# Terascale-All-sensing-Research-Studio/MOV-SLAM

Measured on AMD Instinct MI355X. Metric: local-BA iterations/sec (50 KF x 20k MapPoint window), higher is better.
Workload: dtype f64; 1 GPU; LocalBundleAdjustment 50 KF + 10 fixed x 20000 MapPoints, E=110510 mono edges, Huber on, 10 LM iterations (cfg3, seed 1003); one window per GPU; parallelism=1 window

## Files before the change

### mov-slam_amd/csrc/coarse_level.h

```cpp
#pragma once
#include <hip/hip_runtime.h>

#include <type_traits>

#include "device_math.h"
#include "device_types.h"
#include "handoff.h"

namespace movba {

#ifndef MOVBA_COARSE_EXTRAPOLATE
#define MOVBA_COARSE_EXTRAPOLATE 1
#endif

template <int kT, int kNC, int kPA>
__device__ __forceinline__ void coarse_build(const DevWindow &w, const PcgParams &pp, int trial, double lambda, double *sm, bool extrapolate)
{
    double *Ac = sm;
    double *gj = Ac + kNC * kNC;
    int &s_bad = *reinterpret_cast<int *>(gj + 9 * kNC + 2);
    const int tid = threadIdx.x;
    const int nf = w.nfree;
#ifdef MOVBA_CLOCK_STAMP
    unsigned long long cst_last = __builtin_amdgcn_s_memtime();
#define COARSE_STAMP(k) do { const unsigned long long _t = __builtin_amdgcn_s_memtime(); if (tid == 0) w.ctrl->dbg_seg2[k] += _t - cst_last; cst_last = _t; } while (0)
#else
#define COARSE_STAMP(k) do { } while (0)
#endif
    const double *part = w.part, *part_ = part;
    double *blocks = w.blocks_c;
    if (tid == 0) s_bad = 0;
    for (int idx = tid; idx < kNC * kNC; idx += kT) Ac[idx] = 0.0;

    const int ndiag = nf * 36;
    for (int idx = tid; idx < w.n_multi * 36; idx += kT) {
        const int m = idx / 36, k = idx - m * 36, pr = w.multi_pairs[m];
        double sacc = 0.0;
        for (int itx = w.pair_item_start[pr]; itx < w.pair_item_start[pr + 1]; ++itx) sacc += part[(size_t)itx * kPartStride + k];
        blocks[pr * 36 + k] = -sacc;
    }
    for (int base = tid; base < ndiag; base += 4 * kT) {
        int k[4], hu[4], i0[4], i1[4];
        double s[4] = { 0, 0, 0, 0 }, hp[4] = { 0, 0, 0, 0 };
        int nmax = 0;
#pragma unroll
        for (int m = 0; m < 4; ++m) {
            const int idx = min(base + m * kT, ndiag - 1);
            const int pr = idx / 36;
            k[m] = idx - pr * 36;
            const int a = k[m] / 6, b = k[m] - a * 6;
            hu[m] = 42 + (a <= b ? ut6(a, b) : ut6(b, a));
            i0[m] = w.pair_item_start[pr]; i1[m] = w.pair_item_start[pr + 1];
            nmax = max(nmax, i1[m] - i0[m]);
        }
        for (int o = 0; o < nmax; o += 6) {
            double sv[4][6], hv[4][6];
#pragma unroll
            for (int m = 0; m < 4; ++m)
#pragma unroll
                for (int u = 0; u < 6; ++u) {
                    const double *src = part + (size_t)min(i0[m] + o + u, i1[m] - 1) * kPartStride;
                    sv[m][u] = src[k[m]]; hv[m][u] = src[hu[m]];
                }
#pragma unroll
            for (int m = 0; m < 4; ++m)
#pragma unroll
                for (int u = 0; u < 6; ++u) { const bool in = i0[m] + o + u < i1[m]; s[m] += in ? sv[m][u] : 0.0; hp[m] += in ? hv[m][u] : 0.0; }
        }
#pragma unroll
        for (int m = 0; m < 4; ++m) {
            const int idx = base + m * kT;
            if (idx < ndiag) blocks[idx] = (hp[m] + ((k[m] % 7 == 0) ? lambda : 0.0)) - s[m];
        }
    }
    __syncthreads();
    COARSE_STAMP(2);
    double *aggc = gj;
    if (tid < kNC / kPA) {
        const int g0 = pp.wave_row0[tid], g1 = pp.wave_row0[tid + 1];
        aggc[tid] = g0 + 0.5 * (g1 - g0 - 1); aggc[kNC / kPA + tid] = 1.0 / fmax(1.0, 0.5 * (g1 - g0));
    }
    int *tent = reinterpret_cast<int *>(gj + 9 * kNC + 8), *tij = tent + w.cblk_ptr[w.n_cblk];
    for (int q = tid; q < w.cblk_ptr[w.n_cblk]; q += kT) { tent[q] = w.cblk_ent[q]; tij[q] = w.cblk_ij[q]; }
    __syncthreads();
    const int nw = w.n_cblk * 6;
    const bool split = 2 * nw <= kT;
    auto walk = [&](int cb, int a, int part, double (&s00)[6], double (&s01)[6], double (&s10)[6], double (&s11)[6]) {
        const int g = w.cblk_g[cb], h = w.cblk_h[cb];
        const double cg = aggc[g], ch = aggc[h], ig = aggc[kNC / kPA + g], ih = aggc[kNC / kPA + h];
        int t0 = w.cblk_ptr[cb], t1 = w.cblk_ptr[cb + 1];
        if (split) {
            const int n = t1 - t0, front = min(n, (((n + 1) >> 1) + 7) & ~7);
            if (part == 0) t1 = t0 + front; else t0 += front;
        }
#pragma unroll
        for (int m = 0; m < 6; ++m) s00[m] = s01[m] = s10[m] = s11[m] = 0.0;
        for (int t = t0; t < t1; t += 8) {
            int pk[8], ij[8];
            double v[8][6];
#pragma unroll
            for (int u = 0; u < 8; ++u) { const int tt = min(t + u, t1 - 1); pk[u] = tent[tt]; ij[u] = tij[tt]; }
#pragma unroll
            for (int u = 0; u < 8; ++u) {
                const int e = pk[u];
                const double *src = (e & 1) ? part_ + (size_t)(e >> 2) * kPartStride : blocks + (size_t)(e >> 2) * 36;
                const int o0 = (e & 2) ? a : a * 6, st = (e & 2) ? 6 : 1;
#pragma unroll
                for (int m = 0; m < 6; ++m) v[u][m] = src[o0 + st * m];
            }
#pragma unroll
            for (int u = 0; u < 8; ++u) {
                const bool in = t + u < t1;
                const double sgn = in ? ((pk[u] & 1) ? -1.0 : 1.0) : 0.0;
                const double pi = ((ij[u] >> 16) - cg) * ig, pj = ((ij[u] & 0xffff) - ch) * ih;
#pragma unroll
                for (int m = 0; m < 6; ++m) {
                    const double x = sgn * v[u][m];
                    s00[m] += x; s01[m] += pj * x; s10[m] += pi * x; s11[m] += pi * pj * x;
                }
            }
        }
        return Ac + (g * kPA + a) * kNC + h * kPA;
    };
    if (split) {
        const bool active = tid < 2 * nw;
        const int half = tid >= nw, wi = tid - half * nw;
        double s00[6], s01[6], s10[6], s11[6];
        double *dst = nullptr;
        if (active) dst = walk(wi / 6, wi - (wi / 6) * 6, half, s00, s01, s10, s11);
        if (active && !half) {
#pragma unroll
            for (int m = 0; m < 6; ++m) { dst[m] = s00[m]; dst[6 + m] = s01[m]; dst[6 * kNC + m] = s10[m]; dst[6 * kNC + 6 + m] = s11[m]; }
        }
        __syncthreads();
        if (active && half) {
#pragma unroll
            for (int m = 0; m < 6; ++m) { dst[m] += s00[m]; dst[6 + m] += s01[m]; dst[6 * kNC + m] += s10[m]; dst[6 * kNC + 6 + m] += s11[m]; }
        }
    } else {
        for (int wi = tid; wi < nw; wi += kT) {
            double s00[6], s01[6], s10[6], s11[6];
            double *dst = walk(wi / 6, wi - (wi / 6) * 6, 0, s00, s01, s10, s11);
#pragma unroll
            for (int m = 0; m < 6; ++m) { dst[m] = s00[m]; dst[6 + m] = s01[m]; dst[6 * kNC + m] = s10[m]; dst[6 * kNC + 6 + m] = s11[m]; }
        }
    }
    __syncthreads();
    if (tid < kNC) {
        const int g = tid / kPA, d = (tid - g * kPA) / 6, nrows = pp.wave_row0[g + 1] - pp.wave_row0[g];
        if (nrows == 0 || (d == 1 && nrows < 2)) {
            for (int j = 0; j < kNC; ++j) { Ac[tid * kNC + j] = 0.0; Ac[j * kNC + tid] = 0.0; }
        }
    }
    __syncthreads();
    if (tid < kNC) {
        const int g = tid / kPA, d = (tid - g * kPA) / 6, nrows = pp.wave_row0[g + 1] - pp.wave_row0[g];
        if (nrows == 0 || (d == 1 && nrows < 2)) Ac[tid * kNC + tid] = 1.0;
    }
    __syncthreads();
    if (extrapolate) {
        double *prev = w.ac_prev;
        const double lam_prev = prev[kNC * kNC], trial_prev = prev[kNC * kNC + 1];
        double gamma = 0.0;
        if (trial >= 1 && trial_prev == (double)(trial - 1) && lambda != lam_prev && MOVBA_COARSE_EXTRAPOLATE) {
            gamma = (lambda * (1.0 / 3.0) - lambda) / (lambda - lam_prev);
            gamma = fmin(fmax(gamma, -1.0), 1.0 / 3.0);
            if (!isfinite(gamma)) gamma = 0.0;
        }
        constexpr int kPer = kNC * kNC / kT;
        static_assert(kPer * kT == kNC * kNC, "one pass");
        double pv[kPer];
#pragma unroll
        for (int u = 0; u < kPer; ++u) pv[u] = prev[tid + u * kT];
        __syncthreads();
#pragma unroll
        for (int u = 0; u < kPer; ++u) {
            const double a = Ac[tid + u * kT];
            prev[tid + u * kT] = a;
            if (gamma != 0.0) Ac[tid + u * kT] = a + gamma * (a - pv[u]);
        }
        if (tid == 0) { prev[kNC * kNC] = lambda; prev[kNC * kNC + 1] = (double)trial; }
        __syncthreads();
    }

    COARSE_STAMP(3);
    static_assert(kNC == 96 && kT == 512, "tile layout written for 96 x 96 on 512 threads");
    double *dsc = gj + 8 * kNC + 2;
    double *pvs = gj + 8 * kNC;
    if (tid < kNC) { const double d = Ac[tid * kNC + tid]; dsc[tid] = (d > 0.0 && isfinite(d)) ? rsqrt(d) : 0.0; if (!(d > 0.0) || !isfinite(d)) s_bad = 1; }
    __syncthreads();
    const int rg = tid >> 4, cg = tid & 15;
    double t[3][6];
#pragma unroll
    for (int r = 0; r < 3; ++r)
#pragma unroll
        for (int q = 0; q < 6; ++q) t[r][q] = Ac[(3 * rg + r) * kNC + 6 * cg + q] * dsc[3 * rg + r] * dsc[6 * cg + q];
    unsigned live = 0;
    for (int q = 0; q < kNC / 6; ++q) {
        const int nrows = pp.wave_row0[(q >> 1) + 1] - pp.wave_row0[q >> 1];
        if (!(nrows == 0 || ((q & 1) && nrows < 2))) live |= 1u << q;
    }
    __syncthreads();
    auto publish = [&](auto Ctag, int gq, int buf) {
        constexpr int C = decltype(Ctag)::value;
        constexpr int lr0 = C % 3, lr1 = (C + 1) % 3;
        const int rg0 = 2 * gq + C / 3, rg1 = 2 * gq + (C + 1) / 3;
        double *R1 = gj + buf * 4 * kNC, *C1 = R1 + kNC, *R2 = C1 + kNC, *C2 = R2 + kNC;
        if (rg == rg0) {
#pragma unroll
            for (int q = 0; q < 6; ++q) R1[6 * cg + q] = t[lr0][q] + ((cg == gq && q == C) ? 1.0 : 0.0);
        }
        if (rg == rg1) {
#pragma unroll
            for (int q = 0; q < 6; ++q) R2[6 * cg + q] = t[lr1][q];
        }
        if (cg == gq) {
#pragma unroll
            for (int r = 0; r < 3; ++r) { C1[3 * rg + r] = t[r][C] - ((rg == rg0 && r == lr0) ? 1.0 : 0.0); C2[3 * rg + r] = t[r][C + 1]; }
        }
        if (rg == rg0 && cg == gq) pvs[buf] = t[lr0][C];
    };
    int kk = live ? __builtin_ctz(live) : kNC / 6;
    if (kk < kNC / 6) publish(std::integral_constant<int, 0>{}, kk, 0);
    __syncthreads();
    bool bad = s_bad != 0;
    int buf = 0;
    auto pair_step = [&](auto Ctag, int gq) -> bool {
        constexpr int C = decltype(Ctag)::value;
        constexpr int lr1 = (C + 1) % 3;
        const int k = 6 * gq + C, rg1 = 2 * gq + (C + 1) / 3;
        const double *R1 = gj + buf * 4 * kNC, *C1 = R1 + kNC, *R2 = C1 + kNC, *C2 = R2 + kNC;
        const double p1 = pvs[buf];
        const double o12 = R1[k + 1], o21 = C1[k + 1], q22 = R2[k + 1];
        double r1[6], r2[6], c1[3], c2[3];
#pragma unroll
        for (int q = 0; q < 6; ++q) { r1[q] = R1[6 * cg + q]; r2[q] = R2[6 * cg + q]; }
#pragma unroll
        for (int r = 0; r < 3; ++r) { c1[r] = C1[3 * rg + r]; c2[r] = C2[3 * rg + r]; }
        if (!(p1 > 0.0) || !isfinite(p1)) return false;
        double ip1 = __builtin_amdgcn_rcp(p1);
        ip1 = ip1 * (2.0 - p1 * ip1);
        ip1 = ip1 * (2.0 - p1 * ip1);
        const double s12 = o12 * ip1;
        const double p2 = q22 - o21 * s12;
        if (!(p2 > 0.0) || !isfinite(p2)) return false;
        double ip2 = __builtin_amdgcn_rcp(p2);
        ip2 = ip2 * (2.0 - p2 * ip2);
        ip2 = ip2 * (2.0 - p2 * ip2);
#pragma unroll
        for (int q = 0; q < 6; ++q) {
            r1[q] *= ip1;
            r2[q] = ((r2[q] - o21 * r1[q]) + ((cg == gq && q == C + 1) ? 1.0 : 0.0)) * ip2;
        }
#pragma unroll
        for (int r = 0; r < 3; ++r) c2[r] = (c2[r] - c1[r] * s12) - ((rg == rg1 && r == lr1) ? 1.0 : 0.0);
#pragma unroll
        for (int r = 0; r < 3; ++r)
#pragma unroll
            for (int q = 0; q < 6; ++q) { t[r][q] -= c1[r] * r1[q]; t[r][q] -= c2[r] * r2[q]; }
        return true;
    };
    while (kk < kNC / 6 && !bad) {
        const unsigned later = kk < 31 ? (live & ~((2u << kk) - 1u)) : 0u;
        const int next = later ? __builtin_ctz(later) : kNC / 6;
        if (!pair_step(std::integral_constant<int, 0>{}, kk)) { bad = true; break; }
        publish(std::integral_constant<int, 2>{}, kk, buf ^ 1);
        __syncthreads(); buf ^= 1;
        if (!pair_step(std::integral_constant<int, 2>{}, kk)) { bad = true; break; }
        publish(std::integral_constant<int, 4>{}, kk, buf ^ 1);
        __syncthreads(); buf ^= 1;
        if (!pair_step(std::integral_constant<int, 4>{}, kk)) { bad = true; break; }
        if (next < kNC / 6) publish(std::integral_constant<int, 0>{}, next, buf ^ 1);
        __syncthreads(); buf ^= 1;
        kk = next;
    }
    if (bad && tid == 0) s_bad = 1;
    __syncthreads();
    COARSE_STAMP(4);
    float *dst = w.aci + (size_t)(trial & 1) * kNC * kNC;
#pragma unroll
    for (int r = 0; r < 3; ++r)
#pragma unroll
        for (int q = 0; q < 6; ++q) dst[(3 * rg + r) * kNC + 6 * cg + q] = (float)(t[r][q] * dsc[3 * rg + r] * dsc[6 * cg + q]);
    __syncthreads();
    if (tid == 0) w.aci_tag[trial & 1] = s_bad ? -1 : trial;
    COARSE_STAMP(5);
}

}
```

### mov-slam_amd/csrc/pcg_kernel.hip

```cpp
#include <hip/hip_runtime.h>

#include "coarse_level.h"
#include "device_math.h"
#include "device_types.h"
#include "handoff.h"
#include "kernels.h"

namespace movba {

#ifdef MOVBA_CLOCK_STAMP
#define SEG_STAMP(k) do { unsigned long long _t; asm volatile("s_memtime %0\n\ts_waitcnt lgkmcnt(0)" : "=s"(_t) :: "memory"); seg[k] += _t - seg_last; seg_last = _t; } while (0)
#else
#define SEG_STAMP(k) do { } while (0)
#endif
#ifdef MOVBA_CLOCK_STAMP
#define SETUP_STAMP(k) do { const unsigned long long _t = __builtin_amdgcn_s_memtime(); if (tid == 0) c->dbg_seg2[k] += _t - setup_last; setup_last = _t; } while (0)
#else
#define SETUP_STAMP(k) do { } while (0)
#endif

#ifdef MOVBA_PCG_NO_UNIFORM
#define PCG_UNI(x) (x)
#else
#define PCG_UNI(x) uniform_f64(x)
#endif

namespace {

constexpr int kT = kPcgRowsThreads;
constexpr int kNW = kT / 64;
constexpr int kOwnBatch = 10;
constexpr int kPA = kCoarsePerAgg;
constexpr int kNC = kPA * kNW;
static_assert(kNC == kCoarseDim, "coarse dimension");

__device__ __forceinline__ double sum_fixed(const double *red)
{
    static_assert(kNW == 8, "tree written for 8 waves");
    const double2 *r2 = reinterpret_cast<const double2 *>(red);
    const double2 a = r2[0], b = r2[1], c = r2[2], d = r2[3];
    return ((a.x + a.y) + (b.x + b.y)) + ((c.x + c.y) + (d.x + d.y));
}

}

template <bool OVERFLOW, bool PADDED>
__device__ __forceinline__ void pcg_rows_body(const DevWindow &w, const PcgParams &pp, int trial, int role)
{
    static_assert(!(OVERFLOW && PADDED), "the padded layout holds the register-resident pairs only");
    extern __shared__ __attribute__((aligned(16))) double sm[];
    Ctrl *c = w.ctrl;
    const int tid = threadIdx.x, ln = tid & 63;
    const int wv = __builtin_amdgcn_readfirstlane(tid >> 6);
    const bool fresh = pp.use_coarse == 2;
    const bool solver = role == 0 && !fresh;
    const int nf = w.nfree, n = 6 * nf;
    const int b0 = pp.wave_row0[wv], b1 = pp.wave_row0[wv + 1];
    const int row = b0 * 6 + ln;
    const bool owner = ln < 6 * (b1 - b0);
    const int bi = owner ? row / 6 : 0, ba = owner ? row - bi * 6 : 0;
    const int ctrial = fresh ? trial : trial - 1;
    int cur = 0;
    double lambda = 0.0;
#ifdef MOVBA_CLOCK_STAMP
    const unsigned long long stamp_c0 = __builtin_amdgcn_s_memtime(), stamp_t0 = __builtin_amdgcn_s_memrealtime();
    unsigned long long setup_last = stamp_c0;
#endif
    const double *part = w.part;
    if (!solver) {
        if (c->done) return;
        cur = c->cur; lambda = c->lambda;
        if (role == 1) {
            coarse_build<kT, kNC, kPA>(w, pp, trial, lambda, sm, true);
            return;
        }
        coarse_build<kT, kNC, kPA>(w, pp, trial, lambda, sm, false);
        __syncthreads();
    }
    int done_w = 0;
    if (solver) { done_w = c->done; cur = c->cur; lambda = c->lambda; }
    int aci_tag = -1;
    if (pp.use_coarse) {
        typedef __attribute__((address_space(1))) const void *gptr_t;
        typedef __attribute__((address_space(3))) void *lptr_t;
        const int npad0 = (6 * w.nfree + 1) & ~1;
        float *acf0 = reinterpret_cast<float *>(sm + 2 * npad0 + 36 * w.nfree + 2 * kNW + 2);
        aci_tag = w.aci_tag[max(ctrial, 0) & 1];
        const float *src = w.aci + (size_t)(max(ctrial, 0) & 1) * kNC * kNC;
        static_assert((kNC * kNC) % 256 == 0, "whole waves of 16-byte pieces");
#pragma unroll
        for (int u = 0; u * kT * 4 < kNC * kNC; ++u) {
            const int piece = tid + u * kT;
            if ((piece & ~63) * 4 < kNC * kNC)
                __builtin_amdgcn_global_load_lds((gptr_t)(src + 4 * piece), (lptr_t)(acf0 + 4 * (piece & ~63)), 16, 0, 0);
        }
    }
    const int4 *plan = reinterpret_cast<const int4 *>(w.lane_plan) + (size_t)tid * 3;
    const int4 pl0 = plan[0], pl1 = plan[1], plo = plan[2];
    const int oi0 = plo.x, oi1 = plo.y;
    const int rp_b0 = pp.wave_ent0[wv], rp_b1 = pp.wave_ent0[wv + 1], rp_nf = pp.nrowent, rp_bi = plo.z, rp_bi1 = plo.w;
    constexpr int kRecFly = 4;
    double2 rv[kRecFly][4];
    const double2 *rec0 = reinterpret_cast<const double2 *>(w.rec_d + (size_t)bi * w.rec_slots * 48 + ba * 8);
#pragma unroll
    for (int u = 0; u < kRecFly; ++u) {
        const double2 *src = rec0 + (size_t)min(u, w.rec_slots - 1) * 24;
#pragma unroll
        for (int q = 0; q < 4; ++q) rv[u][q] = src[q];
    }
    double Bo[2][36];
    if (!OVERFLOW) {
#pragma unroll
        for (int k = 0; k < 2; ++k)
#pragma unroll
            for (int q = 0; q < 36; ++q) Bo[k][q] = w.img_b[(size_t)(36 * k + q) * kT + tid];
    }
    if (solver && done_w) return;
    SETUP_STAMP(6);
    const int npad = (n + 1) & ~1;
    const int nrowent_all = rp_nf;

    double *p_lds = sm;
    double *r_lds = p_lds + npad;
    double *minv = r_lds + npad;
    double *red0 = minv + 36 * nf;
    double *red1 = red0 + kNW;
    float *Acf = reinterpret_cast<float *>(red1 + kNW + 2);
    double *rcg = red1 + kNW + 2 + kNC * kNC / 2;
    double *zstrip = rcg + kNC + 32 * wv;
    double *ustrip = zstrip + 16;
    double z_reg = 0.0, u_reg = 0.0;
    double *ypart = rcg + kNC + 32 * kNW;
    constexpr int kYDummy = 5 * kOwnBatch + 6;
    const int ypart_len = PADDED ? n * kOwnBatch + kYDummy + kOwnBatch : 6 * ((nrowent_all >> 1) + 1 + kOwnBatch);
    double *sdiag = ypart + ypart_len;
    double *rsw = sdiag + 36 * nf + 64 * wv;
    if (PADDED) {
        for (int k = tid; k < ypart_len; k += kT) ypart[k] = 0.0;
    }
    const int nrowent = nrowent_all;
    const int P0 = rp_b0 >> 1, P1 = rp_b1 >> 1;
    const int own_p0 = rp_bi >> 1, own_p1 = rp_bi1 >> 1;
    const int own_cnt = own_p1 - own_p0;
    const int nb = b1 - b0;

    if (OVERFLOW) {
        const int e0 = 2 * (P0 + 64), ntail = max(2 * P1 - e0, 0) * 36;
        for (int base = ln; base < ntail; base += 8 * 64) {
            int q[8], src[8], hu[8], i0[8], i1[8], pr[8];
            double sv[8], hv[8];
#pragma unroll
            for (int u = 0; u < 8; ++u) {
                const int idx = min(base + 64 * u, ntail - 1);
                const int e = e0 + idx / 36;
                q[u] = idx - (idx / 36) * 36;
                const RowEnt re = w.row_ent[e];
                const int a = q[u] / 6, b = q[u] - a * 6;
                pr[u] = re.block;
                src[u] = re.transposed ? b * 6 + a : q[u];
                hu[u] = 42 + (a <= b ? ut6(a, b) : ut6(b, a));
                i0[u] = re.block >= 0 ? w.pair_item_start[re.block] : 0;
                i1[u] = re.block >= 0 ? w.pair_item_start[re.block + 1] : 0;
            }
#pragma unroll
            for (int u = 0; u < 8; ++u) {
                const double *rec = part + (size_t)i0[u] * kPartStride;
                sv[u] = i1[u] > i0[u] ? rec[src[u]] : 0.0;
                hv[u] = (i1[u] > i0[u] && pr[u] < nf) ? rec[hu[u]] : 0.0;
            }
#pragma unroll
            for (int u = 0; u < 8; ++u)
                for (int itx = i0[u] + 1; itx < i1[u]; ++itx) {
                    const double *rec = part + (size_t)itx * kPartStride;
                    sv[u] += rec[src[u]];
                    if (pr[u] < nf) hv[u] += rec[hu[u]];
                }
#pragma unroll
            for (int u = 0; u < 8; ++u) {
                const int idx = base + 64 * u;
                if (idx < ntail) {
                    const bool dg = pr[u] >= 0 && pr[u] < nf;
                    w.blocks_ov[(size_t)e0 * 36 + idx] = dg ? (hv[u] + (q[u] % 7 == 0 ? lambda : 0.0)) - sv[u] : -sv[u];
                }
            }
        }
        __syncthreads();
    }

    int colo[2];
    const int my_pair = P0 + ln;
    const bool have_pair = my_pair < P1;
    int yslot = (have_pair ? my_pair : (nrowent >> 1)) * 6;
    const double *yown = ypart + own_p0 * 6 + ba;
    if (PADDED) {
        yslot = n * kOwnBatch;
#pragma unroll
        for (int u = 0; u < 10; ++u) {
            const int q0 = __builtin_amdgcn_readlane(rp_bi, 6 * u) >> 1, q1 = __builtin_amdgcn_readlane(rp_bi1, 6 * u) >> 1;
            if (u < nb && have_pair && my_pair >= q0 && my_pair < q1) yslot = (b0 + u) * 6 * kOwnBatch + (my_pair - q0);
        }
        yown = ypart + (owner ? row : 0) * kOwnBatch;
    }
    double r_r = 0.0;
    double mi[6] = { 1, 1, 1, 1, 1, 1 };
    auto wave_lds_sync0 = [&]() {
        __builtin_amdgcn_fence(__ATOMIC_RELEASE, "wavefront");
        __builtin_amdgcn_wave_barrier();
        __builtin_amdgcn_fence(__ATOMIC_ACQUIRE, "wavefront");
    };
    if (owner) {
        double d6[6] = { 0, 0, 0, 0, 0, 0 }, cc = 0.0, bb = 0.0;
        const int ni = oi1 - oi0;
        auto add = [&](const double2 (&v)[4], bool in) {
            d6[0] += in ? v[0].x : 0.0; d6[1] += in ? v[0].y : 0.0; d6[2] += in ? v[1].x : 0.0;
            d6[3] += in ? v[1].y : 0.0; d6[4] += in ? v[2].x : 0.0; d6[5] += in ? v[2].y : 0.0;
            cc += in ? v[3].x : 0.0; bb += in ? v[3].y : 0.0;
        };
#pragma unroll
        for (int u = 0; u < kRecFly; ++u) add(rv[u], u < ni);
        for (int i0 = kRecFly; i0 < ni; i0 += kRecFly) {
            double2 v[kRecFly][4];
#pragma unroll
            for (int u = 0; u < kRecFly; ++u) {
                const double2 *src = rec0 + (size_t)min(i0 + u, ni - 1) * 24;
#pragma unroll
                for (int q = 0; q < 4; ++q) v[u][q] = src[q];
            }
#pragma unroll
            for (int u = 0; u < kRecFly; ++u) add(v[u], i0 + u < ni);
        }
#pragma unroll
        for (int q = 0; q < 6; ++q) d6[q] += q == ba ? lambda : 0.0;
#pragma unroll
        for (int q = 0; q < 6; ++q) sdiag[bi * 36 + ba * 6 + q] = d6[q];
        r_r = bb - cc;
        w.bp[row] = bb;
#pragma unroll
        for (int q = 0; q < 6; ++q) mi[q] = d6[q];
    }
    SETUP_STAMP(7);
    {
        bool bad = false;
#pragma unroll
        for (int k = 0; k < 6; ++k) {
            double *strip = ((k & 1) ? p_lds : r_lds) + (owner ? bi * 6 : 0);
            if (owner && ba == k) {
                const double p = mi[k];
                if (!(p > 0.0)) bad = true;
                double pinv = __builtin_amdgcn_rcp(p);
                pinv = pinv * (2.0 - p * pinv);
                pinv = pinv * (2.0 - p * pinv);
#pragma unroll
                for (int q = 0; q < 6; ++q) { mi[q] = q == k ? pinv : mi[q] * pinv; strip[q] = mi[q]; }
            }
            wave_lds_sync0();
            if (owner && ba != k) {
                const double2 *sr = reinterpret_cast<const double2 *>(strip);
                const double2 s0 = sr[0], s1 = sr[1], s2 = sr[2];
                const double srow[6] = { s0.x, s0.y, s1.x, s1.y, s2.x, s2.y };
                const double f = mi[k];
#pragma unroll
                for (int q = 0; q < 6; ++q) mi[q] = q == k ? -f * srow[k] : mi[q] - f * srow[q];
            }
        }
        if (owner) {
#pragma unroll
            for (int q = 0; q < 6; ++q) minv[bi * 36 + ba * 6 + q] = mi[q];
        }
        wave_lds_sync0();
        if (owner) {
            double col[6];
#pragma unroll
            for (int q = 0; q < 6; ++q) col[q] = minv[bi * 36 + q * 6 + ba];
#pragma unroll
            for (int q = 0; q < 6; ++q) mi[q] = 0.5 * (mi[q] + col[q]);
        }
        wave_lds_sync0();
        if (owner) {
#pragma unroll
            for (int q = 0; q < 6; ++q) minv[bi * 36 + ba * 6 + q] = mi[q];
        }
        const int wbad = __any(bad) ? 1 : 0;
        if (ln == 0) reinterpret_cast<int *>(red1)[wv] = wbad;
    }
    const bool coarse = pp.use_coarse && ctrial >= 0 && aci_tag == ctrial;
    SETUP_STAMP(0);
    wave_lds_sync0();

#pragma unroll
    for (int k = 0; k < 2; ++k) {
        colo[k] = 0;
        const int4 pl = k ? pl1 : pl0;
        const bool valid = pl.x >= 0, tr = valid && ((pl.y >> 30) & 1) != 0;
        if (valid) colo[k] = pl.y & 0x3fffffff;
        const bool diag = valid && pl.x < nf, from_img = !OVERFLOW && valid && pl.x >= nf && pl.w - pl.z == 1;
        if (!OVERFLOW) {
#pragma unroll
            for (int q = 0; q < 36; ++q) Bo[k][q] = from_img ? -Bo[k][q] : 0.0;
        } else {
#pragma unroll
            for (int q = 0; q < 36; ++q) Bo[k][q] = 0.0;
        }
        if (diag) {
            const double2 *src = reinterpret_cast<const double2 *>(sdiag + pl.x * 36);
#pragma unroll
            for (int q = 0; q < 18; ++q) { const double2 v = src[q]; Bo[k][2 * q] = v.x; Bo[k][2 * q + 1] = v.y; }
        }
        if (__any(valid && !diag && !from_img)) {
            double raw[36];
#pragma unroll
            for (int q = 0; q < 36; ++q) raw[q] = 0.0;
            const bool mine = valid && !diag && !from_img;
            for (int itx = mine ? pl.z : 0; itx < (mine ? pl.w : 0); ++itx) {
                const double2 *src = reinterpret_cast<const double2 *>(part + (size_t)itx * kPartStride);
#pragma unroll
                for (int q = 0; q < 18; ++q) { const double2 v = src[q]; raw[2 * q] -= v.x; raw[2 * q + 1] -= v.y; }
            }
#pragma unroll
            for (int a = 0; a < 6; ++a)
#pragma unroll
                for (int q = 0; q < 6; ++q) Bo[k][a * 6 + q] = mine ? (tr ? raw[q * 6 + a] : raw[a * 6 + q]) : Bo[k][a * 6 + q];
        }
    }
    SETUP_STAMP(1);

    double x_r = 0.0, z_r = 0.0;
    const double2 *mrow = reinterpret_cast<const double2 *>(minv + (owner ? bi * 36 + ba * 6 : 0));
    const double2 *rblk = reinterpret_cast<const double2 *>(PADDED ? rsw + (owner ? (bi - b0) * 6 : 0) : r_lds + (owner ? bi * 6 : 0));
    auto wave_lds_sync = [&]() {
        __builtin_amdgcn_fence(__ATOMIC_RELEASE, "wavefront");
        __builtin_amdgcn_wave_barrier();
        __builtin_amdgcn_fence(__ATOMIC_ACQUIRE, "wavefront");
    };
    const double agg_c = uniform_f64(b0 + 0.5 * (nb - 1)), agg_ih = uniform_f64(1.0 / fmax(1.0, 0.5 * nb));
    const double agg_cc = uniform_f64(0.5 * (nb - 1));
    const double phi = owner ? (bi - agg_c) * agg_ih : 0.0;
    const int crow = min(ln >> 2, kPA - 1), cq = ln & 3;
    auto restrict_own = [&](double v_r) {
        if (PADDED) rsw[ln] = owner ? v_r : 0.0;
        else if (owner) r_lds[row] = v_r;
        wave_lds_sync();
        if (ln < kPA) {
            const int a = ln < 6 ? ln : ln - 6;
            const double *rb = PADDED ? rsw + a : r_lds + b0 * 6 + a;
            double v[10];
#pragma unroll
            for (int u = 0; u < 10; ++u) v[u] = rb[6 * u];
            if (!PADDED) {
#pragma unroll
                for (int u = 0; u < 10; ++u) v[u] = (u < nb) ? v[u] : 0.0;
            }
            const double tc = (((v[0] + v[1]) + (v[2] + v[3])) + ((v[4] + v[5]) + (v[6] + v[7]))) + (v[8] + v[9]);
            const double ti = (((v[1] + 2.0 * v[2]) + (3.0 * v[3] + 4.0 * v[4])) + ((5.0 * v[5] + 6.0 * v[6]) + (7.0 * v[7] + 8.0 * v[8]))) + 9.0 * v[9];
            rcg[wv * kPA + ln] = ln < 6 ? tc : (ti - agg_cc * tc) * agg_ih;
        }
    };
    const int ra = ln < kPA ? (ln < 6 ? ln : ln - 6) : 0;
    auto restrict_issue = [&](double v_r, double (&v)[10]) {
        if (PADDED) rsw[ln] = owner ? v_r : 0.0;
        else if (owner) r_lds[row] = v_r;
        wave_lds_sync();
        const double *rb = PADDED ? rsw + ra : r_lds + b0 * 6 + ra;
#pragma unroll
        for (int u = 0; u < 10; ++u) v[u] = rb[6 * u];
    };
    auto restrict_finish = [&](double (&v)[10]) {
        if (ln < kPA) {
            if (!PADDED) {
#pragma unroll
                for (int u = 0; u < 10; ++u) v[u] = (u < nb) ? v[u] : 0.0;
            }
            const double tc = (((v[0] + v[1]) + (v[2] + v[3])) + ((v[4] + v[5]) + (v[6] + v[7]))) + (v[8] + v[9]);
            const double ti = (((v[1] + 2.0 * v[2]) + (3.0 * v[3] + 4.0 * v[4])) + ((5.0 * v[5] + 6.0 * v[6]) + (7.0 * v[7] + 8.0 * v[8]))) + 9.0 * v[9];
            rcg[wv * kPA + ln] = ln < 6 ? tc : (ti - agg_cc * tc) * agg_ih;
        }
    };
    auto coarse_rows = [&]() {
        const float4 *arow = reinterpret_cast<const float4 *>(Acf + (wv * kPA + crow) * kNC + cq * 24);
        const double2 *rcv = reinterpret_cast<const double2 *>(rcg + cq * 24);
        double t0 = 0.0, t1 = 0.0;
#pragma unroll
        for (int q = 0; q < 6; q += 2) {
            const float4 a0 = arow[q], a1 = arow[q + 1];
            const double2 c0 = rcv[2 * q], c1 = rcv[2 * q + 1], c2 = rcv[2 * q + 2], c3 = rcv[2 * q + 3];
            t0 += ((double)a0.x * c0.x + (double)a0.y * c0.y) + ((double)a0.z * c1.x + (double)a0.w * c1.y);
            t1 += ((double)a1.x * c2.x + (double)a1.y * c2.y) + ((double)a1.z * c3.x + (double)a1.w * c3.y);
        }
        double t = t0 + t1;
        t += dpp_mov0<0xb1>(t);
        t += dpp_mov0<0x4e>(t);
        return t;
    };
    if (coarse) {
        restrict_own(r_r);
        u_reg = 0.0;
        __syncthreads();
        const double t = coarse_rows();
        z_reg = t;
        __syncthreads();
    } else __syncthreads();
    int anybad = 0;
#pragma unroll
    for (int k = 0; k < kNW; ++k) anybad |= reinterpret_cast<const int *>(red1)[k];
    auto precond = [&](double rv) {
        if (PADDED) rsw[ln] = owner ? rv : 0.0;
        else if (owner) r_lds[row] = rv;
        wave_lds_sync();
        const double2 m0 = mrow[0], m1 = mrow[1], m2 = mrow[2];
        const double2 r0 = rblk[0], r1 = rblk[1], r2 = rblk[2];
        double s = (m0.x * r0.x + m0.y * r0.y) + (m1.x * r1.x + m1.y * r1.y) + (m2.x * r2.x + m2.y * r2.y);
        if (fresh && coarse) s = 0.0;
        if (coarse) {
            const double zc0 = __shfl(z_reg, 4 * ba), zc1 = __shfl(z_reg, 24 + 4 * ba);
            if (owner) s += zc0 + phi * zc1;
        }
        return owner ? s : 0.0;
    };
    double p_r = 0.0, s_r = 0.0;
    double inv_gamma = 1.0, inv_alpha = 0.0, alpha = 0.0, thresh = 0.0;
    bool fail = anybad != 0;
    bool first = true;
    int iters = 0;
    int stop = 0;

#ifdef MOVBA_CLOCK_STAMP
    unsigned long long seg[8] = { 0, 0, 0, 0, 0, 0, 0, 0 }, seg_last = __builtin_amdgcn_s_memtime();
#endif
    if (!fail) {
        for (iters = 1; iters <= pp.max_iters; ++iters) {
            if (stop) break;
            SEG_STAMP(7);
            x_r += alpha * p_r;
            r_r -= alpha * s_r;
            if (coarse) {
                if ((iters & 63) == 0) {
                    __syncthreads();
                    restrict_own(r_r);
                    __syncthreads();
                    const double zc = coarse_rows();
                    z_reg = zc;
                    __syncthreads();
                } else z_reg -= alpha * u_reg;
            }
            z_r = precond(r_r);
            if (owner) p_lds[row] = z_r;
            SEG_STAMP(0);
            __syncthreads();
            SEG_STAMP(1);
            {
                const double2 *pa = reinterpret_cast<const double2 *>(p_lds + colo[0]);
                const double2 *pb = reinterpret_cast<const double2 *>(p_lds + colo[1]);
                const double2 a0 = pa[0], a1 = pa[1], a2 = pa[2], c0 = pb[0], c1 = pb[1], c2 = pb[2];
                double y[6];
#pragma unroll
                for (int a = 0; a < 6; ++a)
                    y[a] = Bo[0][a * 6] * a0.x + Bo[0][a * 6 + 1] * a0.y + Bo[0][a * 6 + 2] * a1.x + Bo[0][a * 6 + 3] * a1.y +
                           Bo[0][a * 6 + 4] * a2.x + Bo[0][a * 6 + 5] * a2.y +
                           Bo[1][a * 6] * c0.x + Bo[1][a * 6 + 1] * c0.y + Bo[1][a * 6 + 2] * c1.x + Bo[1][a * 6 + 3] * c1.y +
                           Bo[1][a * 6 + 4] * c2.x + Bo[1][a * 6 + 5] * c2.y;
                if (PADDED) {
                    double *yo = ypart + yslot;
#pragma unroll
                    for (int a = 0; a < 6; ++a) yo[a * kOwnBatch] = y[a];
                } else {
                    double2 *yo = reinterpret_cast<double2 *>(ypart + yslot);
                    yo[0] = make_double2(y[0], y[1]); yo[1] = make_double2(y[2], y[3]); yo[2] = make_double2(y[4], y[5]);
                }
            }
            if (OVERFLOW) for (int pq = P0 + ln + 64; pq < P1; pq += 64) {
                const int c0 = w.row_ent[2 * pq].col * 6, c1 = w.row_ent[2 * pq + 1].col * 6;
                const double2 *B = reinterpret_cast<const double2 *>(w.blocks_ov + (size_t)(2 * pq) * 36);
                const double2 *pa = reinterpret_cast<const double2 *>(p_lds + c0);
                const double2 *pb = reinterpret_cast<const double2 *>(p_lds + c1);
                const double2 a0 = pa[0], a1 = pa[1], a2 = pa[2], c0v = pb[0], c1v = pb[1], c2v = pb[2];
                double y[6];
#pragma unroll
                for (int a = 0; a < 6; ++a) {
                    const double2 u0 = B[3 * a], u1 = B[3 * a + 1], u2 = B[3 * a + 2];
                    const double2 v0 = B[18 + 3 * a], v1 = B[18 + 3 * a + 1], v2 = B[18 + 3 * a + 2];
                    y[a] = (u0.x * a0.x + u0.y * a0.y + u1.x * a1.x + u1.y * a1.y + u2.x * a2.x + u2.y * a2.y) +
                           (v0.x * c0v.x + v0.y * c0v.y + v1.x * c1v.x + v1.y * c1v.y + v2.x * c2v.x + v2.y * c2v.y);
                }
                double2 *yo = reinterpret_cast<double2 *>(ypart + pq * 6);
                yo[0] = make_double2(y[0], y[1]); yo[1] = make_double2(y[2], y[3]); yo[2] = make_double2(y[4], y[5]);
            }
            SEG_STAMP(2);
            wave_lds_sync();
            double w_r = 0.0;
            if (PADDED) {
                const double2 *yb = reinterpret_cast<const double2 *>(yown);
                const double2 v0 = yb[0], v1 = yb[1], v2 = yb[2], v3 = yb[3], v4 = yb[4];
                static_assert(kOwnBatch == 10, "tree written for 10");
                w_r += (((v0.x + v0.y) + (v1.x + v1.y)) + ((v2.x + v2.y) + (v3.x + v3.y))) + (v4.x + v4.y);
                w_r = owner ? w_r : 0.0;
            } else {
                const double *yb = yown;
                for (int e = 0; e < own_cnt; e += kOwnBatch, yb += 6 * kOwnBatch) {
                    double v[kOwnBatch];
#pragma unroll
                    for (int u = 0; u < kOwnBatch; ++u) v[u] = yb[6 * u];
#pragma unroll
                    for (int u = 0; u < kOwnBatch; ++u) v[u] = (e + u < own_cnt) ? v[u] : 0.0;
                    static_assert(kOwnBatch == 10, "tree written for 10");
                    w_r += (((v[0] + v[1]) + (v[2] + v[3])) + ((v[4] + v[5]) + (v[6] + v[7]))) + (v[8] + v[9]);
                }
            }
            SEG_STAMP(3);
            double rv10[10];
            if (coarse) restrict_issue(w_r, rv10);
            {
                double g = owner ? r_r * z_r : 0.0, d = owner ? w_r * z_r : 0.0;
                wave_sum_dpp2(g, d);
                if (ln == 0) *reinterpret_cast<double2 *>(red0 + 2 * wv) = make_double2(g, d);
            }
            if (coarse) restrict_finish(rv10);
            SEG_STAMP(4);
            __syncthreads();
            SEG_STAMP(5);
            double g, delta;
            {
                const double2 gd = *reinterpret_cast<const double2 *>(red0 + 2 * (ln & 7));
                double a = gd.x, b = gd.y;
                a += dpp_mov0<0xb1>(a); b += dpp_mov0<0xb1>(b);
                a += dpp_mov0<0x4e>(a); b += dpp_mov0<0x4e>(b);
                a += dpp_mov0<0x141>(a); b += dpp_mov0<0x141>(b);
                g = PCG_UNI(a); delta = PCG_UNI(b);
            }
            const double yc = coarse ? coarse_rows() : 0.0;
#ifdef MOVBA_PCG_EARLY_CHECKS
            if (!isfinite(g) || !isfinite(delta)) { stop = 1; ++iters; break; }
            if (first) {
                thresh = PCG_UNI(pp.rel_tol * pp.rel_tol * g);
                if (!(g >= 0.0)) { stop = 1; ++iters; break; }
                if (g == 0.0) { stop = 3; ++iters; break; }
            }
            if (!first && g <= thresh) { stop = 2; ++iters; break; }
            const double beta = PCG_UNI(first ? 0.0 : g * inv_gamma);
            const double den = delta - beta * g * inv_alpha;
            if (!(den > 0.0)) { stop = 1; ++iters; break; }
#else
            if (first) thresh = PCG_UNI(pp.rel_tol * pp.rel_tol * g);
            const double beta = PCG_UNI(first ? 0.0 : g * inv_gamma);
            const double den = delta - beta * g * inv_alpha;
            {
                const bool nonfin = !(isfinite(g) && isfinite(delta));
                const bool neg = first && !(g >= 0.0), zero = first && g == 0.0, conv = !first && g <= thresh, noden = !(den > 0.0);
                stop = (nonfin || neg) ? 1 : zero ? 3 : conv ? 2 : noden ? 1 : 0;
            }
#endif
            inv_gamma = PCG_UNI(fast_rcp(g));
            alpha = PCG_UNI(g * fast_rcp(den));
            inv_alpha = PCG_UNI(den * inv_gamma);
            first = false;
            p_r = z_r + beta * p_r;
            s_r = w_r + beta * s_r;
            if (coarse) {
                u_reg = yc + beta * u_reg;
                wave_lds_sync();
            }
            SEG_STAMP(6);
        }
    }
    if (stop) { iters = stop == 3 ? 0 : iters - 1; fail = stop == 1; }
    const bool capped = iters > pp.max_iters;
    if (capped) iters = pp.max_iters;
    double T0[7] = { 0, 0, 0, 1, 0, 0, 0 };
    int h0 = -1;
    if (tid < w.NP) {
#pragma unroll
        for (int k = 0; k < 7; ++k) T0[k] = w.st[cur].pose[7 * tid + k];
        h0 = w.hidx[tid];
    }
    __syncthreads();
    if (fail || capped) {
        if (tid == 0) {
            const int np = c->n_pause + 1;
            c->pcg_last_iters = iters;
            c->pcg_total_iters += iters;
            c->solver_mode = 1; c->direct_from = c->n_solves;
            c->n_pause = np;
            c->done = 2;
            __hip_atomic_store(&w.hstat->pause_seq, np, __ATOMIC_RELAXED, __HIP_MEMORY_SCOPE_SYSTEM);
        }
        return;
    }

    const double xv = owner ? x_r : 0.0;
    if (owner) { w.xp[row] = xv; p_lds[row] = xv; }
    {
        const double ps = wave_sum_dpp(owner ? xv * (lambda * xv + w.bp[row]) : 0.0);
        if (ln == 0) red0[wv] = ps;
    }
    __syncthreads();
    const double scs = sum_fixed(red0);
    const DevState &S0 = w.st[cur];
    const DevState &S1 = w.st[cur ^ 1];
    for (int i = tid; i < w.NP; i += kT) {
        double T[7];
#pragma unroll
        for (int k = 0; k < 7; ++k) T[k] = i == tid ? T0[k] : S0.pose[7 * i + k];
        const int h = i == tid ? h0 : w.hidx[i];
        store_trial_pose(S1.pose, S1.Rt, i, T, h, true, p_lds);
    }
#ifdef MOVBA_CLOCK_STAMP
    if (ln == 0) for (int k = 0; k < 8; ++k) c->dbg_wseg[wv][k] += seg[k];
#endif
    if (tid == 0) {
        w.scale_part[w.n_pt_blocks] = scs;
        c->pcg_fail = 0;
        c->pcg_last_iters = iters;
        c->pcg_total_iters += iters;
#ifdef MOVBA_CLOCK_STAMP
        c->dbg_cycles += __builtin_amdgcn_s_memtime() - stamp_c0;
        c->dbg_ticks += __builtin_amdgcn_s_memrealtime() - stamp_t0;
        for (int k = 0; k < 8; ++k) c->dbg_seg[k] += seg[k];
        (void)setup_last;
#endif
    }
}

template <bool OVERFLOW, bool PADDED>
__global__ __launch_bounds__(kT) void k_pcg_rows(DevWindow w, PcgParams pp, int trial) { pcg_rows_body<OVERFLOW, PADDED>(w, pp, trial, blockIdx.x); }

template <bool OVERFLOW, bool PADDED>
__global__ __launch_bounds__(kT) void k_pcg_rows_b(BatchDev b, int trial)
{
    const int wi = blockIdx.x >> 1, role = blockIdx.x & 1;
    const PcgParams &pp = b.pps[wi];
    if (b.band_bw && b.band_bw[wi] >= 0) return;
    if (role == 1 && pp.use_coarse != 1) return;
    pcg_rows_body<OVERFLOW, PADDED>(b.wins[wi], pp, trial, role);
}

static_assert(kNW == kPcgPlanWaves && kNC == kCoarseDim && kOwnBatch == kPcgPlanOwnBatch, "pcg_plan.cpp sizes the LDS carve of this kernel");

hipError_t launch_pcg_rows(const DevWindow &w, int nrowent, const PcgParams &pp, int trial, hipStream_t s)
{
    const dim3 g(pp.use_coarse == 1 ? 2 : 1), t(kT);
    const bool padded = pp.padded && !pp.overflow;
    const size_t lds = pcg_rows_lds_bytes(w.nfree, nrowent, padded);
    if (pp.overflow) hipLaunchKernelGGL((k_pcg_rows<true, false>), g, t, lds, s, w, pp, trial);
    else if (padded) hipLaunchKernelGGL((k_pcg_rows<false, true>), g, t, lds, s, w, pp, trial);
    else hipLaunchKernelGGL((k_pcg_rows<false, false>), g, t, lds, s, w, pp, trial);
    return hipGetLastError();
}

hipError_t launch_pcg_rows_batch(const BatchDev &b, bool overflow, bool padded, size_t lds, int trial, hipStream_t s)
{
    if (overflow) hipLaunchKernelGGL((k_pcg_rows_b<true, false>), dim3(2 * b.n), dim3(kT), lds, s, b, trial);
    else if (padded) hipLaunchKernelGGL((k_pcg_rows_b<false, true>), dim3(2 * b.n), dim3(kT), lds, s, b, trial);
    else hipLaunchKernelGGL((k_pcg_rows_b<false, false>), dim3(2 * b.n), dim3(kT), lds, s, b, trial);
    return hipGetLastError();
}

hipError_t configure_pcg_rows()
{
    const void *fs[6] = { reinterpret_cast<const void *>(k_pcg_rows<false, false>), reinterpret_cast<const void *>(k_pcg_rows<false, true>),
                          reinterpret_cast<const void *>(k_pcg_rows<true, false>),
                          reinterpret_cast<const void *>(k_pcg_rows_b<false, false>), reinterpret_cast<const void *>(k_pcg_rows_b<false, true>),
                          reinterpret_cast<const void *>(k_pcg_rows_b<true, false>) };
    for (const void *f : fs) {
        const hipError_t e = hipFuncSetAttribute(f, hipFuncAttributeMaxDynamicSharedMemorySize, 160 * 1024 - 1024);
        if (e != hipSuccess) return e;
    }
    return hipSuccess;
}

}
```

Baseline: 9514 LM iterations/s.

## Store coarse inverse in per-lane tile layout matching the product's access pattern

The coarse-level builder now writes the float coarse inverse in a tiled layout where each lane's 3x6 block is contiguous in float4/float2 chunks strided by wave, instead of row-major. The PCG coarse product reads the matching tile with four float4 loads plus one float2, computes three partial row dots, and reduces across 16-lane groups with DPP row shifts. The shuffle source for the coarse correction is remapped to the new lane ownership. This is meant to coalesce the builder's stores and the product's loads and cut redundant reads of the coarse vector, at the cost of a more intricate reduction whose correctness depends on the index mapping.

Result: no change. 9476 LM iterations/s (-0.4%).

```diff
diff --git a/mov-slam_amd/csrc/coarse_level.h b/mov-slam_amd/csrc/coarse_level.h
--- a/mov-slam_amd/csrc/coarse_level.h
+++ b/mov-slam_amd/csrc/coarse_level.h
@@ -12,6 +12,21 @@
 #ifndef MOVBA_COARSE_EXTRAPOLATE
 #define MOVBA_COARSE_EXTRAPOLATE 1
 #endif
+
+constexpr int kAciTileRows = 3, kAciTileCols = 6, kAciTile = kAciTileRows * kAciTileCols;
+constexpr int kAciWave = 64 * kAciTile;
+constexpr int kAciHalves = 64 * 16;
+static_assert(4 * kAciTileRows == kCoarsePerAgg && 16 * kAciTileCols == kCoarseDim && kAciTile == 18, "4 x 16 tiles per aggregate");
+__host__ __device__ inline int aci_tile_index(int g, int lane, int e)
+{
+    return g * kAciWave + (e < 16 ? (e >> 2) * 256 + 4 * lane + (e & 3) : kAciHalves + 2 * lane + (e - 16));
+}
+__host__ __device__ inline int aci_image_index(int row, int col)
+{
+    const int g = row / kCoarsePerAgg, rr = row - g * kCoarsePerAgg, rg = rr / kAciTileRows, r = rr - rg * kAciTileRows;
+    const int cg = col / kAciTileCols, c = col - cg * kAciTileCols;
+    return aci_tile_index(g, 16 * rg + cg, kAciTileCols * r + c);
+}
 
 template <int kT, int kNC, int kPA>
 __device__ __forceinline__ void coarse_build(const DevWindow &w, const PcgParams &pp, int trial, double lambda, double *sm, bool extrapolate)
@@ -277,11 +292,16 @@
     if (bad && tid == 0) s_bad = 1;
     __syncthreads();
     COARSE_STAMP(4);
-    float *dst = w.aci + (size_t)(trial & 1) * kNC * kNC;
+    static_assert(kT == 512 && kPA == kCoarsePerAgg, "the builder's tiles are the product's");
+    float *dst = w.aci + (size_t)(trial & 1) * kNC * kNC + aci_tile_index(tid >> 6, tid & 63, 0);
+    float v[kAciTile];
 #pragma unroll
     for (int r = 0; r < 3; ++r)
 #pragma unroll
-        for (int q = 0; q < 6; ++q) dst[(3 * rg + r) * kNC + 6 * cg + q] = (float)(t[r][q] * dsc[3 * rg + r] * dsc[6 * cg + q]);
+        for (int q = 0; q < 6; ++q) v[6 * r + q] = (float)(t[r][q] * dsc[3 * rg + r] * dsc[6 * cg + q]);
+#pragma unroll
+    for (int p = 0; p < 4; ++p) *reinterpret_cast<float4 *>(dst + 256 * p) = make_float4(v[4 * p], v[4 * p + 1], v[4 * p + 2], v[4 * p + 3]);
+    *reinterpret_cast<float2 *>(w.aci + (size_t)(trial & 1) * kNC * kNC + aci_tile_index(tid >> 6, tid & 63, 16)) = make_float2(v[16], v[17]);
     __syncthreads();
     if (tid == 0) w.aci_tag[trial & 1] = s_bad ? -1 : trial;
     COARSE_STAMP(5);
diff --git a/mov-slam_amd/csrc/pcg_kernel.hip b/mov-slam_amd/csrc/pcg_kernel.hip
--- a/mov-slam_amd/csrc/pcg_kernel.hip
+++ b/mov-slam_amd/csrc/pcg_kernel.hip
@@ -335,7 +335,6 @@
     const double agg_c = uniform_f64(b0 + 0.5 * (nb - 1)), agg_ih = uniform_f64(1.0 / fmax(1.0, 0.5 * nb));
     const double agg_cc = uniform_f64(0.5 * (nb - 1));
     const double phi = owner ? (bi - agg_c) * agg_ih : 0.0;
-    const int crow = min(ln >> 2, kPA - 1), cq = ln & 3;
     auto restrict_own = [&](double v_r) {
         if (PADDED) rsw[ln] = owner ? v_r : 0.0;
         else if (owner) r_lds[row] = v_r;
@@ -376,19 +375,21 @@
         }
     };
     auto coarse_rows = [&]() {
-        const float4 *arow = reinterpret_cast<const float4 *>(Acf + (wv * kPA + crow) * kNC + cq * 24);
-        const double2 *rcv = reinterpret_cast<const double2 *>(rcg + cq * 24);
-        double t0 = 0.0, t1 = 0.0;
-#pragma unroll
-        for (int q = 0; q < 6; q += 2) {
-            const float4 a0 = arow[q], a1 = arow[q + 1];
-            const double2 c0 = rcv[2 * q], c1 = rcv[2 * q + 1], c2 = rcv[2 * q + 2], c3 = rcv[2 * q + 3];
-            t0 += ((double)a0.x * c0.x + (double)a0.y * c0.y) + ((double)a0.z * c1.x + (double)a0.w * c1.y);
-            t1 += ((double)a1.x * c2.x + (double)a1.y * c2.y) + ((double)a1.z * c3.x + (double)a1.w * c3.y);
-        }
-        double t = t0 + t1;
-        t += dpp_mov0<0xb1>(t);
-        t += dpp_mov0<0x4e>(t);
+        const float *tile = Acf + aci_tile_index(wv, ln, 0);
+        const float4 a0 = *reinterpret_cast<const float4 *>(tile), a1 = *reinterpret_cast<const float4 *>(tile + 256);
+        const float4 a2 = *reinterpret_cast<const float4 *>(tile + 512), a3 = *reinterpret_cast<const float4 *>(tile + 768);
+        const float2 a4 = *reinterpret_cast<const float2 *>(Acf + aci_tile_index(wv, ln, 16));
+        const double2 *rcv = reinterpret_cast<const double2 *>(rcg + kAciTileCols * (ln & 15));
+        const double2 c0 = rcv[0], c1 = rcv[1], c2 = rcv[2];
+        double t0 = ((double)a0.x * c0.x + (double)a0.y * c0.y) + ((double)a0.z * c1.x + (double)a0.w * c1.y) + ((double)a1.x * c2.x + (double)a1.y * c2.y);
+        double t1 = ((double)a1.z * c0.x + (double)a1.w * c0.y) + ((double)a2.x * c1.x + (double)a2.y * c1.y) + ((double)a2.z * c2.x + (double)a2.w * c2.y);
+        double t2 = ((double)a3.x * c0.x + (double)a3.y * c0.y) + ((double)a3.z * c1.x + (double)a3.w * c1.y) + ((double)a4.x * c2.x + (double)a4.y * c2.y);
+        t0 += dpp_mov0<0xb1>(t0);  t1 += dpp_mov0<0xb1>(t1);  t2 += dpp_mov0<0xb1>(t2);
+        t0 += dpp_mov0<0x4e>(t0);  t1 += dpp_mov0<0x4e>(t1);  t2 += dpp_mov0<0x4e>(t2);
+        const int qp = ln & 3;
+        double t = qp == 0 ? t0 : qp == 1 ? t1 : t2;
+        t += dpp_mov0<0x124>(t);
+        t += dpp_mov0<0x128>(t);
         return t;
     };
     if (coarse) {
@@ -411,7 +412,8 @@
         double s = (m0.x * r0.x + m0.y * r0.y) + (m1.x * r1.x + m1.y * r1.y) + (m2.x * r2.x + m2.y * r2.y);
         if (fresh && coarse) s = 0.0;
         if (coarse) {
-            const double zc0 = __shfl(z_reg, 4 * ba), zc1 = __shfl(z_reg, 24 + 4 * ba);
+            const int zsrc = 16 * (ba / 3) + ba % 3;
+            const double zc0 = __shfl(z_reg, zsrc), zc1 = __shfl(z_reg, 32 + zsrc);
             if (owner) s += zc0 + phi * zc1;
         }
         return owner ? s : 0.0;
```
